# zhengfei0908/SBA-GAN

Hardware: AMD Instinct MI355X
Metric: images/sec (G+D step) at 256px (higher is better)
Workload: dtype bf16; 1 GPU; bird_style.yml 3-stage G+D step (64..256px), B=20 per GPU, G_NET variant=model, image_encoder=inception, text_encoder=RNN_ENCODER in the step; global_batch=20, parallelism=dp1, launch=replayer, losses_finite=True

## Files before the change

sba-gan_amd/csrc/encoder.hip:

```cpp
#include "common.h"

namespace {

__global__ void resize_fwd_kernel(const float* __restrict__ in, float* __restrict__ out, int NC, int S, int D) {
    const int64_t total = (int64_t)NC * D * D;
    const float sc = (float)(S - 1) / (float)(D - 1);
    for (int64_t i = blockIdx.x * (int64_t)blockDim.x + threadIdx.x; i < total; i += (int64_t)gridDim.x * blockDim.x) {
        const int x = (int)(i % D), y = (int)((i / D) % D);
        const int64_t nc = i / ((int64_t)D * D);
        const float fy = y * sc, fx = x * sc;
        int y0 = (int)fy, x0 = (int)fx;
        y0 = min(y0, S - 1); x0 = min(x0, S - 1);
        const int y1 = min(y0 + 1, S - 1), x1 = min(x0 + 1, S - 1);
        const float wy = fy - y0, wx = fx - x0;
        const float* p = in + nc * S * S;
        const float v = (1.f - wy) * ((1.f - wx) * p[y0 * S + x0] + wx * p[y0 * S + x1]) +
                        wy * ((1.f - wx) * p[y1 * S + x0] + wx * p[y1 * S + x1]);
        out[i] = v;
    }
}

__device__ __forceinline__ float resize_adj_w(int o, int r, float sc, int S) {
    const float f = o * sc;
    int i0 = (int)f;
    i0 = min(i0, S - 1);
    const int i1 = min(i0 + 1, S - 1);
    const float wgt = f - i0;
    return (i0 == r ? 1.f - wgt : 0.f) + (i1 == r ? wgt : 0.f);
}

__global__ void resize_bwd_kernel(const float* __restrict__ dout, float* __restrict__ din, int NC, int S, int D) {
    const int64_t total = (int64_t)NC * S * S;
    const float sc = (float)(S - 1) / (float)(D - 1);
    const float inv = 1.f / sc;
    for (int64_t i = blockIdx.x * (int64_t)blockDim.x + threadIdx.x; i < total; i += (int64_t)gridDim.x * blockDim.x) {
        const int c = (int)(i % S), r = (int)((i / S) % S);
        const int64_t nc = i / ((int64_t)S * S);
        const int ylo = max(0, (int)floorf((r - 1) * inv) - 1), yhi = min(D - 1, (int)ceilf((r + 1) * inv) + 1);
        const int xlo = max(0, (int)floorf((c - 1) * inv) - 1), xhi = min(D - 1, (int)ceilf((c + 1) * inv) + 1);
        const float* g = dout + nc * D * D;
        float acc = 0.f;
        for (int y = ylo; y <= yhi; ++y) {
            const float wy = resize_adj_w(y, r, sc, S);
            if (wy == 0.f) continue;
            float row = 0.f;
            for (int x = xlo; x <= xhi; ++x) {
                const float wx = resize_adj_w(x, c, sc, S);
                if (wx != 0.f) row += g[y * D + x] * wx;
            }
            acc += wy * row;
        }
        din[i] = acc;
    }
}

constexpr int RESIZE_MAXC = 4;
__global__ __launch_bounds__(256) void resize_bwd_tab_kernel(const float* __restrict__ dout, float* __restrict__ din, int NC,
                                                             int S, int D) {
    extern __shared__ unsigned char rs_lds[];
    int* t_o = reinterpret_cast<int*>(rs_lds);
    float* t_w = reinterpret_cast<float*>(rs_lds + (size_t)S * RESIZE_MAXC * 4);
    const float sc = (float)(S - 1) / (float)(D - 1);
    const float inv = 1.f / sc;
    for (int r = threadIdx.x; r < S; r += blockDim.x) {
        const int lo = max(0, (int)floorf((r - 1) * inv) - 1), hi = min(D - 1, (int)ceilf((r + 1) * inv) + 1);
        int k = 0;
        for (int o = lo; o <= hi && k < RESIZE_MAXC; ++o) {
            const float wgt = resize_adj_w(o, r, sc, S);
            if (wgt != 0.f) { t_o[r * RESIZE_MAXC + k] = o; t_w[r * RESIZE_MAXC + k] = wgt; ++k; }
        }
        for (; k < RESIZE_MAXC; ++k) { t_o[r * RESIZE_MAXC + k] = 0; t_w[r * RESIZE_MAXC + k] = 0.f; }
    }
    __syncthreads();
    const int64_t total = (int64_t)NC * S * S;
    for (int64_t i = blockIdx.x * (int64_t)blockDim.x + threadIdx.x; i < total; i += (int64_t)gridDim.x * blockDim.x) {
        const int c = (int)(i % S), r = (int)((i / S) % S);
        const int64_t nc = i / ((int64_t)S * S);
        const float* g = dout + nc * D * D;
        float acc = 0.f;
#pragma unroll
        for (int ky = 0; ky < RESIZE_MAXC; ++ky) {
            const float wy = t_w[r * RESIZE_MAXC + ky];
            if (wy == 0.f) continue;
            const float* grow = g + t_o[r * RESIZE_MAXC + ky] * D;
            float row = 0.f;
#pragma unroll
            for (int kx = 0; kx < RESIZE_MAXC; ++kx) {
                const float wx = t_w[c * RESIZE_MAXC + kx];
                if (wx != 0.f) row += grow[t_o[c * RESIZE_MAXC + kx]] * wx;
            }
            acc += wy * row;
        }
        din[i] = acc;
    }
}

template <typename T>
__global__ __launch_bounds__(256) void enc_stem_fwd_kernel(const float* __restrict__ img, const float* __restrict__ w,
                                                           const float* __restrict__ bias, T* __restrict__ out,
                                                           int N, int S, int O, int C) {
    constexpr int V = Vec16<T>::N;
    extern __shared__ float s_w[];
    for (int i = threadIdx.x; i < 27 * C; i += blockDim.x) {
        const int co = i / 27, k = i - co * 27;
        s_w[k * C + co] = w[i];
    }
    __syncthreads();
    const int cv = C / V;
    const int64_t total = (int64_t)N * O * O * cv;
    for (int64_t i = blockIdx.x * (int64_t)blockDim.x + threadIdx.x; i < total; i += (int64_t)gridDim.x * blockDim.x) {
        const int c = (int)(i % cv) * V;
        const int64_t p = i / cv;
        const int ox = (int)(p % O), oy = (int)((p / O) % O), n = (int)(p / ((int64_t)O * O));
        float acc[V];
#pragma unroll
        for (int k = 0; k < V; ++k) acc[k] = bias ? bias[c + k] : 0.f;
#pragma unroll
        for (int kh = 0; kh < 3; ++kh)
#pragma unroll
            for (int kw = 0; kw < 3; ++kw)
#pragma unroll
                for (int ci = 0; ci < 3; ++ci) {
                    const float v = img[(((int64_t)n * 3 + ci) * S + 2 * oy + kh) * S + 2 * ox + kw];
                    const float* wr = &s_w[((kh * 3 + kw) * 3 + ci) * C + c];
#pragma unroll
                    for (int k = 0; k < V; ++k) acc[k] += v * wr[k];
                }
        Vec16<T> o;
#pragma unroll
        for (int k = 0; k < V; ++k) o.set(k, bias ? fmaxf(acc[k], 0.f) : acc[k]);
        st16(out + p * C + c, o);
    }
}

template <typename T>
__global__ __launch_bounds__(256) void enc_stem_resize_fwd_kernel(const float* __restrict__ img, const float* __restrict__ w,
                                                                  const float* __restrict__ bias, T* __restrict__ out,
                                                                  int N, int S, int D, int O, int C) {
    constexpr int V = Vec16<T>::N;
    extern __shared__ float s_w[];
    for (int i = threadIdx.x; i < 27 * C; i += blockDim.x) {
        const int co = i / 27, k = i - co * 27;
        s_w[k * C + co] = w[i];
    }
    __syncthreads();
    const float sc = (float)(S - 1) / (float)(D - 1);
    const int cv = C / V;
    const int64_t total = (int64_t)N * O * O * cv;
    for (int64_t i = blockIdx.x * (int64_t)blockDim.x + threadIdx.x; i < total; i += (int64_t)gridDim.x * blockDim.x) {
        const int c = (int)(i % cv) * V;
        const int64_t p = i / cv;
        const int ox = (int)(p % O), oy = (int)((p / O) % O), n = (int)(p / ((int64_t)O * O));
        int x0[3], x1[3];
        float wx[3];
#pragma unroll
        for (int k = 0; k < 3; ++k) {
            const float fx = (2 * ox + k) * sc;
            x0[k] = min((int)fx, S - 1);
            x1[k] = min(x0[k] + 1, S - 1);
            wx[k] = fx - x0[k];
        }
        float acc[V];
#pragma unroll
        for (int k = 0; k < V; ++k) acc[k] = bias ? bias[c + k] : 0.f;
        const float* q0 = img + (int64_t)n * 3 * S * S;
#pragma unroll 1
        for (int kh = 0; kh < 3; ++kh) {
            const float fy = (2 * oy + kh) * sc;
            const int y0 = min((int)fy, S - 1), y1 = min(y0 + 1, S - 1);
            const float wy = fy - y0;
#pragma unroll
            for (int kw = 0; kw < 3; ++kw)
#pragma unroll
                for (int ci = 0; ci < 3; ++ci) {
                    const float* q = q0 + (int64_t)ci * S * S;
                    const float v = (1.f - wy) * ((1.f - wx[kw]) * q[y0 * S + x0[kw]] + wx[kw] * q[y0 * S + x1[kw]]) +
                                    wy * ((1.f - wx[kw]) * q[y1 * S + x0[kw]] + wx[kw] * q[y1 * S + x1[kw]]);
                    const float* wr = &s_w[((kh * 3 + kw) * 3 + ci) * C + c];
#pragma unroll
                    for (int k = 0; k < V; ++k) acc[k] += v * wr[k];
                }
        }
        Vec16<T> o;
#pragma unroll
        for (int k = 0; k < V; ++k) o.set(k, bias ? fmaxf(acc[k], 0.f) : acc[k]);
        st16(out + p * C + c, o);
    }
}

template <typename T>
__global__ __launch_bounds__(256) void enc_stem_bwd_kernel(const float* __restrict__ w, const T* __restrict__ out,
                                                           const T* __restrict__ dout, float* __restrict__ dimg,
                                                           int N, int S, int O, int C) {
    constexpr int V = Vec16<T>::N;
    extern __shared__ float s_w[];
    for (int i = threadIdx.x; i < 27 * C; i += blockDim.x) {
        const int co = i / 27, k = i - co * 27;
        s_w[k * C + co] = w[i];
    }
    __syncthreads();
    const int64_t total = (int64_t)N * S * S;
    for (int64_t p = blockIdx.x * (int64_t)blockDim.x + threadIdx.x; p < total; p += (int64_t)gridDim.x * blockDim.x) {
        const int ix = (int)(p % S), iy = (int)((p / S) % S), n = (int)(p / ((int64_t)S * S));
        float acc[3] = {0.f, 0.f, 0.f};
        for (int kh = iy & 1; kh < 3; kh += 2) {
            const int oy = (iy - kh) >> 1;
            if (iy - kh < 0 || oy >= O) continue;
            for (int kw = ix & 1; kw < 3; kw += 2) {
                const int ox = (ix - kw) >> 1;
                if (ix - kw < 0 || ox >= O) continue;
                const int64_t q = (((int64_t)n * O + oy) * O + ox) * C;
                for (int cv = 0; cv < C / V; ++cv) {
                    Vec16<T> ov = ld16(out + q + cv * V), dv = ld16(dout + q + cv * V);
#pragma unroll
                    for (int k = 0; k < V; ++k) {
                        const float dp = ov.get(k) > 0.f ? dv.get(k) : 0.f;
                        const int co = cv * V + k;
#pragma unroll
                        for (int ci = 0; ci < 3; ++ci) acc[ci] += dp * s_w[((kh * 3 + kw) * 3 + ci) * C + co];
                    }
                }
            }
        }
#pragma unroll
        for (int ci = 0; ci < 3; ++ci) dimg[(((int64_t)n * 3 + ci) * S + iy) * S + ix] = acc[ci];
    }
}

__global__ __launch_bounds__(256) void enc_stem_bwd_mfma_kernel(const float* __restrict__ w, const bf16_t* __restrict__ out,
                                                                const bf16_t* __restrict__ dout, float* __restrict__ dimg,
                                                                const int N, const int S, const int O, const int ntiles) {
    constexpr int C = 32;
    const int tid = threadIdx.x, lane = tid & 63, wid = tid >> 6;
    const int m = lane & 15, g = lane >> 4;
    bf16x8_t a_hi[4], a_lo[4];
    {
        const int ci = m >> 2, a = (m >> 1) & 1, b = m & 1;
#pragma unroll
        for (int t = 0; t < 4; ++t) {
            const int kh = a + 2 * (t >> 1), kw = b + 2 * (t & 1);
            const bool ok = m < 12 && kh < 3 && kw < 3;
            bf16x8_t hi, lo;
#pragma unroll
            for (int j = 0; j < 8; ++j) {
                const int co = 8 * g + j;
                const float v = ok ? w[co * 27 + (kh * 3 + kw) * 3 + ci] : 0.f;
                const bf16_t h = f2bf(v);
                hi[j] = (short)h;
                lo[j] = (short)f2bf(v - bf2f(h));
            }
            a_hi[t] = hi;
            a_lo[t] = lo;
        }
    }
    const int BH = (S + 1) / 2, tiles_x = (BH + 15) / 16;
    for (int tile = blockIdx.x * 4 + wid; tile < ntiles; tile += gridDim.x * 4) {
        const int txi = tile % tiles_x, by = (tile / tiles_x) % BH, n = tile / (tiles_x * BH);
        const int bx = txi * 16 + m;
        f32x4_t acc = f32x4_t{0.f, 0.f, 0.f, 0.f};
#pragma unroll
        for (int t = 0; t < 4; ++t) {
            const int oy = by - (t >> 1), ox = bx - (t & 1);
            uint4 dv = make_uint4(0, 0, 0, 0), ov = make_uint4(0, 0, 0, 0);
            if (oy >= 0 && oy < O && ox >= 0 && ox < O) {
                const int64_t q = (((int64_t)n * O + oy) * O + ox) * C + 8 * g;
                dv = *reinterpret_cast<const uint4*>(dout + q);
                ov = *reinterpret_cast<const uint4*>(out + q);
            }
            const uint32_t d[4] = {dv.x, dv.y, dv.z, dv.w}, o[4] = {ov.x, ov.y, ov.z, ov.w};
            bf16x8_t bfr;
#pragma unroll
            for (int k = 0; k < 4; ++k) {
                const uint32_t lo_ok = ((o[k] & 0x7fffu) != 0u && (o[k] & 0x8000u) == 0u) ? 0x0000ffffu : 0u;
                const uint32_t hi_ok = ((o[k] & 0x7fff0000u) != 0u && (o[k] & 0x80000000u) == 0u) ? 0xffff0000u : 0u;
                const uint32_t v = d[k] & (lo_ok | hi_ok);
                bfr[2 * k] = (short)(v & 0xffffu);
                bfr[2 * k + 1] = (short)(v >> 16);
            }
            acc = __builtin_amdgcn_mfma_f32_16x16x32_bf16(a_lo[t], bfr, acc, 0, 0, 0);
            acc = __builtin_amdgcn_mfma_f32_16x16x32_bf16(a_hi[t], bfr, acc, 0, 0, 0);
        }
        if (g < 3 && bx < BH) {
            float* o0 = dimg + (((int64_t)n * 3 + g) * S + 2 * by) * S + 2 * bx;
            const bool x1 = 2 * bx + 1 < S, y1 = 2 * by + 1 < S;
            o0[0] = acc[0];
            if (x1) o0[1] = acc[1];
            if (y1) {
                o0[S] = acc[2];
                if (x1) o0[S + 1] = acc[3];
            }
        }
    }
}

template <typename T>
__global__ void maxpool_fwd_kernel(const T* __restrict__ x, T* __restrict__ y, int N, int H, int W, int C, int xcs,
                                   int xco, int ycs, int yco) {
    constexpr int V = Vec16<T>::N;
    const int OH = (H - 3) / 2 + 1, OW = (W - 3) / 2 + 1, cv = C / V;
    const int64_t total = (int64_t)N * OH * OW * cv;
    for (int64_t i = blockIdx.x * (int64_t)blockDim.x + threadIdx.x; i < total; i += (int64_t)gridDim.x * blockDim.x) {
        const int c = (int)(i % cv) * V;
        const int64_t p = i / cv;
        const int ox = (int)(p % OW), oy = (int)((p / OW) % OH), n = (int)(p / ((int64_t)OW * OH));
        float m[V];
#pragma unroll
        for (int k = 0; k < V; ++k) m[k] = -INFINITY;
#pragma unroll
        for (int kh = 0; kh < 3; ++kh)
#pragma unroll
            for (int kw = 0; kw < 3; ++kw) {
                Vec16<T> v = ld16(x + (((int64_t)n * H + 2 * oy + kh) * W + 2 * ox + kw) * xcs + xco + c);
#pragma unroll
                for (int k = 0; k < V; ++k) m[k] = fmaxf(m[k], v.get(k));
            }
        Vec16<T> o;
#pragma unroll
        for (int k = 0; k < V; ++k) o.set(k, m[k]);
        st16(y + p * ycs + yco + c, o);
    }
}

template <typename T>
__global__ void maxpool_fwd_arg_kernel(const T* __restrict__ x, T* __restrict__ y, uint8_t* __restrict__ arg, int N,
                                       int H, int W, int C, int xcs, int xco, int ycs, int yco) {
    constexpr int V = Vec16<T>::N;
    const int OH = (H - 3) / 2 + 1, OW = (W - 3) / 2 + 1, cv = C / V;
    const int64_t total = (int64_t)N * OH * OW * cv;
    for (int64_t i = blockIdx.x * (int64_t)blockDim.x + threadIdx.x; i < total; i += (int64_t)gridDim.x * blockDim.x) {
        const int c = (int)(i % cv) * V;
        const int64_t p = i / cv;
        const int ox = (int)(p % OW), oy = (int)((p / OW) % OH), n = (int)(p / ((int64_t)OW * OH));
        float m[V];
        uint8_t a[V];
#pragma unroll
        for (int k = 0; k < V; ++k) { m[k] = -INFINITY; a[k] = 255; }
#pragma unroll
        for (int kh = 0; kh < 3; ++kh)
#pragma unroll
            for (int kw = 0; kw < 3; ++kw) {
                Vec16<T> v = ld16(x + (((int64_t)n * H + 2 * oy + kh) * W + 2 * ox + kw) * xcs + xco + c);
#pragma unroll
                for (int k = 0; k < V; ++k) {
                    const float f = v.get(k);
                    if (f > m[k]) { m[k] = f; a[k] = (uint8_t)(kh * 3 + kw); }
                }
            }
        Vec16<T> o;
#pragma unroll
        for (int k = 0; k < V; ++k) o.set(k, m[k]);
        st16(y + p * ycs + yco + c, o);
        uint8_t* ap = arg + p * C + c;
        if (V == 8) {
            uint2 w;
            w.x = a[0] | (a[1] << 8) | (a[2] << 16) | ((uint32_t)a[3] << 24);
            w.y = a[4] | (a[5] << 8) | (a[6] << 16) | ((uint32_t)a[7] << 24);
            *reinterpret_cast<uint2*>(ap) = w;
        } else {
            *reinterpret_cast<uint32_t*>(ap) = a[0] | (a[1] << 8) | (a[2] << 16) | ((uint32_t)a[3] << 24);
        }
    }
}

template <typename T>
__global__ void maxpool_bwd_arg_kernel(const uint8_t* __restrict__ arg, const T* __restrict__ dy, T* __restrict__ dx,
                                       int N, int H, int W, int C, int dycs, int dyco, int dxcs, int dxco,
                                       int accumulate, const T* __restrict__ relu_mask) {
    constexpr int V = Vec16<T>::N;
    const int OH = (H - 3) / 2 + 1, OW = (W - 3) / 2 + 1, cv = C / V;
    const int64_t total = (int64_t)N * H * W * cv;
    for (int64_t i = blockIdx.x * (int64_t)blockDim.x + threadIdx.x; i < total; i += (int64_t)gridDim.x * blockDim.x) {
        const int c = (int)(i % cv) * V;
        const int64_t p = i / cv;
        const int ix = (int)(p % W), iy = (int)((p / W) % H), n = (int)(p / ((int64_t)W * H));
        float g[V];
#pragma unroll
        for (int k = 0; k < V; ++k) g[k] = 0.f;
        for (int oy = max(0, (iy - 1) >> 1); oy <= min(OH - 1, iy >> 1); ++oy) {
            if (iy - 2 * oy > 2) continue;
            for (int ox = max(0, (ix - 1) >> 1); ox <= min(OW - 1, ix >> 1); ++ox) {
                if (ix - 2 * ox > 2) continue;
                const uint32_t mypos = (uint32_t)((iy - 2 * oy) * 3 + (ix - 2 * ox));
                const int64_t q = ((int64_t)n * OH + oy) * OW + ox;
                uint32_t aw[2] = {0u, 0u};
                if (V == 8) {
                    const uint2 w = *reinterpret_cast<const uint2*>(arg + q * C + c);
                    aw[0] = w.x; aw[1] = w.y;
                } else {
                    aw[0] = *reinterpret_cast<const uint32_t*>(arg + q * C + c);
                }
                Vec16<T> d = ld16(dy + q * dycs + dyco + c);
#pragma unroll
                for (int k = 0; k < V; ++k)
                    if (((aw[k >> 2] >> (8 * (k & 3))) & 255u) == mypos) g[k] += d.get(k);
            }
        }
        T* op = dx + p * dxcs + dxco + c;
        Vec16<T> o;
        if (accumulate) o = ld16(op);
#pragma unroll
        for (int k = 0; k < V; ++k) o.set(k, g[k] + (accumulate ? o.get(k) : 0.f));
        if (relu_mask) {
            const Vec16<T> m = ld16(relu_mask + p * dxcs + dxco + c);
#pragma unroll
            for (int k = 0; k < V; ++k) if (!(m.get(k) > 0.f)) o.set(k, 0.f);
        }
        st16(op, o);
    }
}

template <typename T>
__global__ void maxpool_bwd_kernel(const T* __restrict__ x, const T* __restrict__ dy, T* __restrict__ dx, int N, int H,
                                   int W, int C, int xcs, int xco, int dycs, int dyco, int dxcs, int dxco,
                                   int accumulate) {
    constexpr int V = Vec16<T>::N;
    const int OH = (H - 3) / 2 + 1, OW = (W - 3) / 2 + 1, cv = C / V;
    const int64_t total = (int64_t)N * H * W * cv;
    for (int64_t i = blockIdx.x * (int64_t)blockDim.x + threadIdx.x; i < total; i += (int64_t)gridDim.x * blockDim.x) {
        const int c = (int)(i % cv) * V;
        const int64_t p = i / cv;
        const int ix = (int)(p % W), iy = (int)((p / W) % H), n = (int)(p / ((int64_t)W * H));
        float g[V];
#pragma unroll
        for (int k = 0; k < V; ++k) g[k] = 0.f;
        for (int oy = max(0, (iy - 1) >> 1); oy <= min(OH - 1, iy >> 1); ++oy) {
            if (iy - 2 * oy > 2) continue;
            for (int ox = max(0, (ix - 1) >> 1); ox <= min(OW - 1, ix >> 1); ++ox) {
                if (ix - 2 * ox > 2) continue;
                const int mypos = (iy - 2 * oy) * 3 + (ix - 2 * ox);
                float m[V];
                int arg[V];
#pragma unroll
                for (int k = 0; k < V; ++k) { m[k] = -INFINITY; arg[k] = -1; }
#pragma unroll
                for (int kh = 0; kh < 3; ++kh)
#pragma unroll
                    for (int kw = 0; kw < 3; ++kw) {
                        Vec16<T> v = ld16(x + (((int64_t)n * H + 2 * oy + kh) * W + 2 * ox + kw) * xcs + xco + c);
#pragma unroll
                        for (int k = 0; k < V; ++k) {
                            const float f = v.get(k);
                            if (f > m[k]) { m[k] = f; arg[k] = kh * 3 + kw; }
                        }
                    }
                Vec16<T> d = ld16(dy + (((int64_t)n * OH + oy) * OW + ox) * dycs + dyco + c);
#pragma unroll
                for (int k = 0; k < V; ++k)
                    if (arg[k] == mypos) g[k] += d.get(k);
            }
        }
        T* op = dx + p * dxcs + dxco + c;
        Vec16<T> o;
        if (accumulate) o = ld16(op);
#pragma unroll
        for (int k = 0; k < V; ++k) o.set(k, g[k] + (accumulate ? o.get(k) : 0.f));
        st16(op, o);
    }
}

template <typename T>
__global__ void avgpool3_kernel(const T* __restrict__ x, T* __restrict__ y, int N, int H, int W, int C, int xcs,
                                int xco, int ycs, int yco, int accumulate) {
    constexpr int V = Vec16<T>::N;
    const int cv = C / V;
    const int64_t total = (int64_t)N * H * W * cv;
    for (int64_t i = blockIdx.x * (int64_t)blockDim.x + threadIdx.x; i < total; i += (int64_t)gridDim.x * blockDim.x) {
        const int c = (int)(i % cv) * V;
        const int64_t p = i / cv;
        const int ix = (int)(p % W), iy = (int)((p / W) % H), n = (int)(p / ((int64_t)W * H));
        float s[V];
#pragma unroll
        for (int k = 0; k < V; ++k) s[k] = 0.f;
#pragma unroll
        for (int dy = -1; dy <= 1; ++dy)
#pragma unroll
            for (int dx = -1; dx <= 1; ++dx) {
                const int yy = iy + dy, xx = ix + dx;
                if (yy < 0 || yy >= H || xx < 0 || xx >= W) continue;
                Vec16<T> v = ld16(x + (((int64_t)n * H + yy) * W + xx) * xcs + xco + c);
#pragma unroll
                for (int k = 0; k < V; ++k) s[k] += v.get(k);
            }
        T* op = y + p * ycs + yco + c;
        Vec16<T> o;
        if (accumulate) o = ld16(op);
#pragma unroll
        for (int k = 0; k < V; ++k) o.set(k, s[k] * (1.f / 9.f) + (accumulate ? o.get(k) : 0.f));
        st16(op, o);
    }
}

template <typename T>
__global__ void relu_bwd_kernel(const T* __restrict__ out, const T* __restrict__ dout, T* __restrict__ dpre,
                                int64_t rows, int C, int ocs, int oco, int dcs, int dco) {
    constexpr int V = Vec16<T>::N;
    const int cv = C / V;
    const int64_t total = rows * cv;
    for (int64_t i = blockIdx.x * (int64_t)blockDim.x + threadIdx.x; i < total; i += (int64_t)gridDim.x * blockDim.x) {
        const int c = (int)(i % cv) * V;
        const int64_t r = i / cv;
        Vec16<T> o = ld16(out + r * ocs + oco + c), d = ld16(dout + r * dcs + dco + c), q;
#pragma unroll
        for (int k = 0; k < V; ++k) q.set(k, o.get(k) > 0.f ? d.get(k) : 0.f);
        st16(dpre + r * C + c, q);
    }
}

template <typename T>
__global__ void gap_fwd_kernel(const T* __restrict__ x, float* __restrict__ y, int N, int HW, int C) {
    const int i = blockIdx.x * blockDim.x + threadIdx.x;
    if (i >= N * C) return;
    const int n = i / C, c = i - n * C;
    float s = 0.f;
    for (int p = 0; p < HW; ++p) s += to_f<T>(x[((int64_t)n * HW + p) * C + c]);
    y[i] = s / HW;
}
template <typename T>
__global__ __launch_bounds__(256) void gap_bwd_kernel(const float* __restrict__ dy, T* __restrict__ dx, int N, int HW, int C) {
    constexpr int V = Vec16<T>::N;
    const int cv = C / V;
    const int total = N * HW * cv;
    for (int i = blockIdx.x * blockDim.x + threadIdx.x; i < total; i += gridDim.x * blockDim.x) {
        const int r = i / cv, c = (i - r * cv) * V;
        const int n = r / HW;
        const float* src = dy + (int64_t)n * C + c;
        Vec16<T> q;
#pragma unroll
        for (int k = 0; k < V; ++k) q.set(k, src[k] / HW);
        st16(dx + (int64_t)r * C + c, q);
    }
}

template <typename T>
__global__ void nhwc_to_nchw_kernel(const T* __restrict__ x, float* __restrict__ y, int N, int HW, int C) {
    const int64_t total = (int64_t)N * HW * C;
    for (int64_t i = blockIdx.x * (int64_t)blockDim.x + threadIdx.x; i < total; i += (int64_t)gridDim.x * blockDim.x) {
        const int p = (int)(i % HW), c = (int)((i / HW) % C), n = (int)(i / ((int64_t)HW * C));
        y[i] = to_f<T>(x[((int64_t)n * HW + p) * C + c]);
    }
}
template <typename T>
__global__ void nchw_to_nhwc_kernel(const float* __restrict__ x, T* __restrict__ y, int N, int HW, int C) {
    const int64_t total = (int64_t)N * HW * C;
    for (int64_t i = blockIdx.x * (int64_t)blockDim.x + threadIdx.x; i < total; i += (int64_t)gridDim.x * blockDim.x) {
        const int c = (int)(i % C), p = (int)((i / C) % HW), n = (int)(i / ((int64_t)HW * C));
        y[i] = from_f<T>(x[((int64_t)n * C + c) * HW + p]);
    }
}

inline int grid_for(int64_t items, int cap = 8192) {
    int64_t b = (items + 255) / 256;
    if (b < 1) b = 1;
    return (int)(b > cap ? cap : b);
}
inline bool slice_ok(int dtype, int C, int cs, int co) {
    const int V = dtype == SBA_BF16 ? 8 : 4;
    return C > 0 && C % V == 0 && cs >= C + co && co >= 0 && cs % V == 0 && co % V == 0;
}

}

extern "C" int sba_resize_bilinear(const float* in, float* out, int NC, int S, int D, int backward, void* stream) {
    if (!in || !out || NC <= 0 || S < 2 || D < 2) return SBA_E_ARG;
    hipStream_t st = (hipStream_t)stream;
    if (!backward) {
        SBA_LAUNCH(resize_fwd_kernel, dim3(grid_for((int64_t)NC * D * D)), dim3(256), 0, st, in, out, NC, S, D);
    } else {
        if (D >= S && S >= 2 && S <= 2048 && 2 * (int64_t)(D - 1) <= 3 * (int64_t)(S - 1))
            SBA_LAUNCH(resize_bwd_tab_kernel, dim3(grid_for((int64_t)NC * S * S, 2048)), dim3(256), (size_t)S * RESIZE_MAXC * 8,
                       st, in, out, NC, S, D);
        else
        SBA_LAUNCH(resize_bwd_kernel, dim3(grid_for((int64_t)NC * S * S)), dim3(256), 0, st, in, out, NC, S, D);
    }
    return SBA_CHECK_LAUNCH();
}

extern "C" int sba_enc_stem_fwd(int dtype, const float* img, const float* w, const float* bias, void* out, int N,
                                int S, int C, void* stream) {
    if (!img || !w || !out || N <= 0 || S < 3 || C <= 0 || C % 8 || C > 256) return SBA_E_ARG;
    const int O = (S - 3) / 2 + 1, V = dtype == SBA_BF16 ? 8 : 4;
    SBA_DISPATCH(dtype, SBA_LAUNCH((enc_stem_fwd_kernel<T>), dim3(grid_for((int64_t)N * O * O * (C / V), 4096)),
                                           dim3(256), sizeof(float) * 27 * C, (hipStream_t)stream, img, w, bias,
                                           (T*)out, N, S, O, C));
    return SBA_CHECK_LAUNCH();
}

extern "C" int sba_enc_stem_bwd(int dtype, const float* w, const void* out, const void* dout, float* dimg, int N,
                                int S, int C, void* stream) {
    if (!w || !out || !dout || !dimg || N <= 0 || S < 3 || C <= 0 || C % 8 || C > 256) return SBA_E_ARG;
    const int O = (S - 3) / 2 + 1;
    if (dtype == SBA_BF16 && C == 32 && (((uintptr_t)out | (uintptr_t)dout) & 15) == 0) {
        const int BH = (S + 1) / 2, ntiles = N * BH * ((BH + 15) / 16);
        SBA_LAUNCH(enc_stem_bwd_mfma_kernel, dim3((ntiles + 3) / 4 < 8192 ? (ntiles + 3) / 4 : 8192), dim3(256), 0,
                   (hipStream_t)stream, w, (const bf16_t*)out, (const bf16_t*)dout, dimg, N, S, O, ntiles);
        return SBA_CHECK_LAUNCH();
    }
    SBA_DISPATCH(dtype, SBA_LAUNCH((enc_stem_bwd_kernel<T>), dim3(grid_for((int64_t)N * S * S, 4096)), dim3(256),
                                           sizeof(float) * 27 * C, (hipStream_t)stream, w, (const T*)out,
                                           (const T*)dout, dimg, N, S, O, C));
    return SBA_CHECK_LAUNCH();
}

extern "C" int sba_maxpool3x3s2_fwd(int dtype, const void* x, void* y, int N, int H, int W, int C, int xcs, int xco,
                                    int ycs, int yco, void* stream) {
    if (!x || !y || N <= 0 || H < 3 || W < 3 || !slice_ok(dtype, C, xcs, xco) || !slice_ok(dtype, C, ycs, yco))
        return SBA_E_ARG;
    const int OH = (H - 3) / 2 + 1, OW = (W - 3) / 2 + 1, V = dtype == SBA_BF16 ? 8 : 4;
    SBA_DISPATCH(dtype, SBA_LAUNCH((maxpool_fwd_kernel<T>), dim3(grid_for((int64_t)N * OH * OW * (C / V))),
                                           dim3(256), 0, (hipStream_t)stream, (const T*)x, (T*)y, N, H, W, C, xcs, xco,
                                           ycs, yco));
    return SBA_CHECK_LAUNCH();
}

extern "C" int sba_maxpool3x3s2_bwd(int dtype, const void* x, const void* dy, void* dx, int N, int H, int W, int C,
                                    int xcs, int xco, int dycs, int dyco, int dxcs, int dxco, int accumulate,
                                    void* stream) {
    if (!x || !dy || !dx || N <= 0 || H < 3 || W < 3 || !slice_ok(dtype, C, xcs, xco) ||
        !slice_ok(dtype, C, dycs, dyco) || !slice_ok(dtype, C, dxcs, dxco))
        return SBA_E_ARG;
    const int V = dtype == SBA_BF16 ? 8 : 4;
    SBA_DISPATCH(dtype, SBA_LAUNCH((maxpool_bwd_kernel<T>), dim3(grid_for((int64_t)N * H * W * (C / V))),
                                           dim3(256), 0, (hipStream_t)stream, (const T*)x, (const T*)dy, (T*)dx, N, H,
                                           W, C, xcs, xco, dycs, dyco, dxcs, dxco, accumulate));
    return SBA_CHECK_LAUNCH();
}

extern "C" int sba_maxpool3x3s2_fwd_arg(int dtype, const void* x, void* y, uint8_t* argmax, int N, int H, int W, int C,
                                        int xcs, int xco, int ycs, int yco, void* stream) {
    if (!x || !y || !argmax || N <= 0 || H < 3 || W < 3 || !slice_ok(dtype, C, xcs, xco) || !slice_ok(dtype, C, ycs, yco))
        return SBA_E_ARG;
    const int OH = (H - 3) / 2 + 1, OW = (W - 3) / 2 + 1, V = dtype == SBA_BF16 ? 8 : 4;
    if (((uintptr_t)argmax & 7) != 0) return SBA_E_ARG;
    SBA_DISPATCH(dtype, SBA_LAUNCH((maxpool_fwd_arg_kernel<T>), dim3(grid_for((int64_t)N * OH * OW * (C / V))),
                                           dim3(256), 0, (hipStream_t)stream, (const T*)x, (T*)y, argmax, N, H, W, C,
                                           xcs, xco, ycs, yco));
    return SBA_CHECK_LAUNCH();
}

extern "C" int sba_maxpool3x3s2_bwd_arg(int dtype, const uint8_t* argmax, const void* dy, void* dx, int N, int H, int W,
                                        int C, int dycs, int dyco, int dxcs, int dxco, int accumulate,
                                        const void* relu_mask, void* stream) {
    if (!argmax || !dy || !dx || N <= 0 || H < 3 || W < 3 || !slice_ok(dtype, C, dycs, dyco) ||
        !slice_ok(dtype, C, dxcs, dxco) || ((uintptr_t)argmax & 7) != 0)
        return SBA_E_ARG;
    const int V = dtype == SBA_BF16 ? 8 : 4;
    SBA_DISPATCH(dtype, SBA_LAUNCH((maxpool_bwd_arg_kernel<T>), dim3(grid_for((int64_t)N * H * W * (C / V))),
                                           dim3(256), 0, (hipStream_t)stream, argmax, (const T*)dy, (T*)dx, N, H, W, C,
                                           dycs, dyco, dxcs, dxco, accumulate, (const T*)relu_mask));
    return SBA_CHECK_LAUNCH();
}

extern "C" int sba_enc_stem_resize_fwd(int dtype, const float* img, const float* w, const float* bias, void* out, int N,
                                       int S, int D, int C, void* stream) {
    if (!img || !w || !out || N <= 0 || S < 2 || D < 3 || C <= 0 || C % 8 || C > 256) return SBA_E_ARG;
    const int O = (D - 3) / 2 + 1, V = dtype == SBA_BF16 ? 8 : 4;
    SBA_DISPATCH(dtype, SBA_LAUNCH((enc_stem_resize_fwd_kernel<T>), dim3(grid_for((int64_t)N * O * O * (C / V), 8192)),
                                           dim3(256), sizeof(float) * 27 * C, (hipStream_t)stream, img, w, bias, (T*)out, N,
                                           S, D, O, C));
    return SBA_CHECK_LAUNCH();
}

extern "C" int sba_avgpool3x3(int dtype, const void* x, void* y, int N, int H, int W, int C, int xcs, int xco,
                              int ycs, int yco, int accumulate, void* stream) {
    if (!x || !y || N <= 0 || H <= 0 || W <= 0 || !slice_ok(dtype, C, xcs, xco) || !slice_ok(dtype, C, ycs, yco))
        return SBA_E_ARG;
    const int V = dtype == SBA_BF16 ? 8 : 4;
    SBA_DISPATCH(dtype, SBA_LAUNCH((avgpool3_kernel<T>), dim3(grid_for((int64_t)N * H * W * (C / V))), dim3(256),
                                           0, (hipStream_t)stream, (const T*)x, (T*)y, N, H, W, C, xcs, xco, ycs, yco,
                                           accumulate));
    return SBA_CHECK_LAUNCH();
}

extern "C" int sba_relu_bwd(int dtype, const void* out, const void* dout, void* dpre, int64_t rows, int C, int ocs,
                            int oco, int dcs, int dco, void* stream) {
    if (!out || !dout || !dpre || rows <= 0 || !slice_ok(dtype, C, ocs, oco) || !slice_ok(dtype, C, dcs, dco))
        return SBA_E_ARG;
    const int V = dtype == SBA_BF16 ? 8 : 4;
    SBA_DISPATCH(dtype, SBA_LAUNCH((relu_bwd_kernel<T>), dim3(grid_for(rows * (C / V))), dim3(256), 0,
                                           (hipStream_t)stream, (const T*)out, (const T*)dout, (T*)dpre, rows, C, ocs,
                                           oco, dcs, dco));
    return SBA_CHECK_LAUNCH();
}

extern "C" int sba_global_avgpool(int dtype, void* x, float* y, int N, int HW, int C, int backward, void* stream) {
    if (!x || !y || N <= 0 || HW <= 0 || C <= 0) return SBA_E_ARG;
    if (!backward) {
        SBA_DISPATCH(dtype, SBA_LAUNCH((gap_fwd_kernel<T>), dim3(cdiv((int64_t)N * C, 256)), dim3(256), 0,
                                               (hipStream_t)stream, (const T*)x, y, N, HW, C));
    } else {
        if (C % 8 != 0 || (int64_t)N * HW * C >= (1ll << 31)) return SBA_E_ARG;
        SBA_DISPATCH(dtype, SBA_LAUNCH((gap_bwd_kernel<T>), dim3(grid_for((int64_t)N * HW * C / (dtype == SBA_BF16 ? 8 : 4))), dim3(256), 0,
                                               (hipStream_t)stream, (const float*)y, (T*)x, N, HW, C));
    }
    return SBA_CHECK_LAUNCH();
}

extern "C" int sba_layout_nhwc_nchw(int dtype, void* nhwc, float* nchw, int N, int HW, int C, int to_nhwc, void* stream) {
    if (!nhwc || !nchw || N <= 0 || HW <= 0 || C <= 0) return SBA_E_ARG;
    if (!to_nhwc) {
        SBA_DISPATCH(dtype, SBA_LAUNCH((nhwc_to_nchw_kernel<T>), dim3(grid_for((int64_t)N * HW * C)), dim3(256), 0,
                                               (hipStream_t)stream, (const T*)nhwc, nchw, N, HW, C));
    } else {
        SBA_DISPATCH(dtype, SBA_LAUNCH((nchw_to_nhwc_kernel<T>), dim3(grid_for((int64_t)N * HW * C)), dim3(256), 0,
                                               (hipStream_t)stream, (const float*)nchw, (T*)nhwc, N, HW, C));
    }
    return SBA_CHECK_LAUNCH();
}
```

Baseline: 2097 images/sec.

## Rework encoder pooling, global-avgpool and layout kernels for cheaper indexing and coalescing

Four encoder kernels are rewritten. Maxpool backward now uses a 3D grid over (n, row, width×channel) with incremental index walking instead of 64-bit div/mod, and it loads its four candidate windows directly. Avgpool3 now computes runs of 4 outputs from a shared 3×6 register window so neighbouring loads are reused. Global average pooling becomes vectorized and unrolled, and the NHWC/NCHW layout conversion becomes a shared-memory tiled transpose. The aim is to cut index arithmetic and uncoalesced traffic in the inception encoder, at the cost of more registers and extra grid-shape logic.

```diff
diff --git a/sba-gan_amd/csrc/encoder.hip b/sba-gan_amd/csrc/encoder.hip
--- a/sba-gan_amd/csrc/encoder.hip
+++ b/sba-gan_amd/csrc/encoder.hip
@@ -293,6 +293,26 @@
     }
 }
 
+constexpr int POOL_GRID_X = 256, POOL_GRID_YZ = 65535;
+struct PoolWalk {
+    uint32_t q, c, dq, dc;
+    __device__ __forceinline__ explicit PoolWalk(uint32_t cv) {
+        const uint32_t i = blockIdx.x * blockDim.x + threadIdx.x, st = gridDim.x * blockDim.x;
+        q = i / cv; c = i - q * cv;
+        dq = st / cv; dc = st - dq * cv;
+    }
+    __device__ __forceinline__ void next(uint32_t cv) {
+        q += dq; c += dc;
+        if (c >= cv) { c -= cv; ++q; }
+    }
+};
+template <typename T> __device__ __forceinline__ Vec16<T> zero16() {
+    Vec16<T> r;
+#pragma unroll
+    for (int k = 0; k < Vec16<T>::N; ++k) r.set(k, 0.f);
+    return r;
+}
+
 template <typename T>
 __global__ void maxpool_fwd_kernel(const T* __restrict__ x, T* __restrict__ y, int N, int H, int W, int C, int xcs,
                                    int xco, int ycs, int yco) {
@@ -363,50 +383,66 @@
 }
 
 template <typename T>
-__global__ void maxpool_bwd_arg_kernel(const uint8_t* __restrict__ arg, const T* __restrict__ dy, T* __restrict__ dx,
-                                       int N, int H, int W, int C, int dycs, int dyco, int dxcs, int dxco,
-                                       int accumulate, const T* __restrict__ relu_mask) {
+__global__ __launch_bounds__(256) void maxpool_bwd_arg_kernel(const uint8_t* __restrict__ arg, const T* __restrict__ dy,
+                                                              T* __restrict__ dx, int N, int H, int W, int C, int dycs, int dyco,
+                                                              int dxcs, int dxco, int accumulate, const T* __restrict__ relu_mask) {
     constexpr int V = Vec16<T>::N;
-    const int OH = (H - 3) / 2 + 1, OW = (W - 3) / 2 + 1, cv = C / V;
-    const int64_t total = (int64_t)N * H * W * cv;
-    for (int64_t i = blockIdx.x * (int64_t)blockDim.x + threadIdx.x; i < total; i += (int64_t)gridDim.x * blockDim.x) {
-        const int c = (int)(i % cv) * V;
-        const int64_t p = i / cv;
-        const int ix = (int)(p % W), iy = (int)((p / W) % H), n = (int)(p / ((int64_t)W * H));
-        float g[V];
-#pragma unroll
-        for (int k = 0; k < V; ++k) g[k] = 0.f;
-        for (int oy = max(0, (iy - 1) >> 1); oy <= min(OH - 1, iy >> 1); ++oy) {
-            if (iy - 2 * oy > 2) continue;
-            for (int ox = max(0, (ix - 1) >> 1); ox <= min(OW - 1, ix >> 1); ++ox) {
-                if (ix - 2 * ox > 2) continue;
-                const uint32_t mypos = (uint32_t)((iy - 2 * oy) * 3 + (ix - 2 * ox));
-                const int64_t q = ((int64_t)n * OH + oy) * OW + ox;
-                uint32_t aw[2] = {0u, 0u};
-                if (V == 8) {
-                    const uint2 w = *reinterpret_cast<const uint2*>(arg + q * C + c);
-                    aw[0] = w.x; aw[1] = w.y;
-                } else {
-                    aw[0] = *reinterpret_cast<const uint32_t*>(arg + q * C + c);
+    const int OH = (H - 3) / 2 + 1, OW = (W - 3) / 2 + 1;
+    const uint32_t cv = C / V;
+    for (int n = blockIdx.z; n < N; n += gridDim.z)
+        for (int iy = blockIdx.y; iy < H; iy += gridDim.y) {
+            const int oys[2] = {(iy - 1) >> 1, iy >> 1};
+            const bool yok[2] = {oys[0] >= 0 && oys[0] < OH, (iy & 1) == 0 && oys[1] < OH};
+            for (PoolWalk it(cv); it.q < (uint32_t)W; it.next(cv)) {
+                const int ix = (int)it.q, c = (int)it.c * V;
+                const int oxs[2] = {(ix - 1) >> 1, ix >> 1};
+                const bool xok[2] = {oxs[0] >= 0 && oxs[0] < OW, (ix & 1) == 0 && oxs[1] < OW};
+                uint32_t aw[2][2][2];
+                Vec16<T> d[2][2];
+#pragma unroll
+                for (int a = 0; a < 2; ++a)
+#pragma unroll
+                    for (int b = 0; b < 2; ++b) {
+                        aw[a][b][0] = aw[a][b][1] = 0xffffffffu;
+                        d[a][b] = zero16<T>();
+                        if (yok[a] && xok[b]) {
+                            const int64_t q = ((int64_t)n * OH + oys[a]) * OW + oxs[b];
+                            if (V == 8) {
+                                const uint2 w = *reinterpret_cast<const uint2*>(arg + q * C + c);
+                                aw[a][b][0] = w.x; aw[a][b][1] = w.y;
+                            } else {
+                                aw[a][b][0] = *reinterpret_cast<const uint32_t*>(arg + q * C + c);
+                            }
+                            d[a][b] = ld16(dy + q * dycs + dyco + c);
+                        }
+                    }
+                const int64_t p = ((int64_t)n * H + iy) * W + ix;
+                T* op = dx + p * dxcs + dxco + c;
+                Vec16<T> o = zero16<T>(), m = zero16<T>();
+                if (accumulate) o = ld16(op);
+                if (relu_mask) m = ld16(relu_mask + p * dxcs + dxco + c);
+                float g[V];
+#pragma unroll
+                for (int k = 0; k < V; ++k) g[k] = 0.f;
+#pragma unroll
+                for (int a = 0; a < 2; ++a)
+#pragma unroll
+                    for (int b = 0; b < 2; ++b) {
+                        if (!(yok[a] && xok[b])) continue;
+                        const uint32_t mypos = (uint32_t)((iy - 2 * oys[a]) * 3 + (ix - 2 * oxs[b]));
+#pragma unroll
+                        for (int k = 0; k < V; ++k)
+                            if (((aw[a][b][k >> 2] >> (8 * (k & 3))) & 255u) == mypos) g[k] += d[a][b].get(k);
+                    }
+#pragma unroll
+                for (int k = 0; k < V; ++k) o.set(k, g[k] + (accumulate ? o.get(k) : 0.f));
+                if (relu_mask) {
+#pragma unroll
+                    for (int k = 0; k < V; ++k) if (!(m.get(k) > 0.f)) o.set(k, 0.f);
                 }
-                Vec16<T> d = ld16(dy + q * dycs + dyco + c);
-#pragma unroll
-                for (int k = 0; k < V; ++k)
-                    if (((aw[k >> 2] >> (8 * (k & 3))) & 255u) == mypos) g[k] += d.get(k);
-            }
-        }
-        T* op = dx + p * dxcs + dxco + c;
-        Vec16<T> o;
-        if (accumulate) o = ld16(op);
-#pragma unroll
-        for (int k = 0; k < V; ++k) o.set(k, g[k] + (accumulate ? o.get(k) : 0.f));
-        if (relu_mask) {
-            const Vec16<T> m = ld16(relu_mask + p * dxcs + dxco + c);
-#pragma unroll
-            for (int k = 0; k < V; ++k) if (!(m.get(k) > 0.f)) o.set(k, 0.f);
-        }
-        st16(op, o);
-    }
+                st16(op, o);
+            }
+        }
 }
 
 template <typename T>
@@ -458,36 +494,55 @@
     }
 }
 
-template <typename T>
-__global__ void avgpool3_kernel(const T* __restrict__ x, T* __restrict__ y, int N, int H, int W, int C, int xcs,
-                                int xco, int ycs, int yco, int accumulate) {
-    constexpr int V = Vec16<T>::N;
-    const int cv = C / V;
-    const int64_t total = (int64_t)N * H * W * cv;
-    for (int64_t i = blockIdx.x * (int64_t)blockDim.x + threadIdx.x; i < total; i += (int64_t)gridDim.x * blockDim.x) {
-        const int c = (int)(i % cv) * V;
-        const int64_t p = i / cv;
-        const int ix = (int)(p % W), iy = (int)((p / W) % H), n = (int)(p / ((int64_t)W * H));
-        float s[V];
-#pragma unroll
-        for (int k = 0; k < V; ++k) s[k] = 0.f;
-#pragma unroll
-        for (int dy = -1; dy <= 1; ++dy)
-#pragma unroll
-            for (int dx = -1; dx <= 1; ++dx) {
-                const int yy = iy + dy, xx = ix + dx;
-                if (yy < 0 || yy >= H || xx < 0 || xx >= W) continue;
-                Vec16<T> v = ld16(x + (((int64_t)n * H + yy) * W + xx) * xcs + xco + c);
-#pragma unroll
-                for (int k = 0; k < V; ++k) s[k] += v.get(k);
-            }
-        T* op = y + p * ycs + yco + c;
-        Vec16<T> o;
-        if (accumulate) o = ld16(op);
-#pragma unroll
-        for (int k = 0; k < V; ++k) o.set(k, s[k] * (1.f / 9.f) + (accumulate ? o.get(k) : 0.f));
-        st16(op, o);
-    }
+constexpr int AVG_RUN = 4;
+template <typename T>
+__global__ __launch_bounds__(256) void avgpool3_kernel(const T* __restrict__ x, T* __restrict__ y, int N, int H, int W, int C,
+                                                       int xcs, int xco, int ycs, int yco, int accumulate) {
+    constexpr int V = Vec16<T>::N, R = AVG_RUN;
+    const uint32_t cv = C / V, runs = ((uint32_t)W + R - 1) / R;
+    for (int n = blockIdx.z; n < N; n += gridDim.z)
+        for (int iy = blockIdx.y; iy < H; iy += gridDim.y) {
+            const int64_t row = ((int64_t)n * H + iy) * W;
+            for (PoolWalk it(cv); it.q < runs; it.next(cv)) {
+                const int x0 = (int)it.q * R, c = (int)it.c * V;
+                Vec16<T> v[3][R + 2], old[R];
+#pragma unroll
+                for (int r = 0; r < 3; ++r)
+#pragma unroll
+                    for (int j = 0; j < R + 2; ++j) {
+                        const int yy = iy + r - 1, xx = x0 + j - 1;
+                        v[r][j] = yy >= 0 && yy < H && xx >= 0 && xx < W
+                                      ? ld16(x + (row + (int64_t)(r - 1) * W + xx) * xcs + xco + c) : zero16<T>();
+                    }
+                T* op = y + (row + x0) * ycs + yco + c;
+#pragma unroll
+                for (int j = 0; j < R; ++j) old[j] = accumulate && x0 + j < W ? ld16(op + (int64_t)j * ycs) : zero16<T>();
+                float f[3][R + 2][V];
+#pragma unroll
+                for (int r = 0; r < 3; ++r)
+#pragma unroll
+                    for (int j = 0; j < R + 2; ++j)
+#pragma unroll
+                        for (int k = 0; k < V; ++k) f[r][j][k] = v[r][j].get(k);
+#pragma unroll
+                for (int j = 0; j < R; ++j) {
+                    if (x0 + j >= W) break;
+                    float s[V];
+#pragma unroll
+                    for (int k = 0; k < V; ++k) s[k] = 0.f;
+#pragma unroll
+                    for (int r = 0; r < 3; ++r)
+#pragma unroll
+                        for (int d = 0; d < 3; ++d)
+#pragma unroll
+                            for (int k = 0; k < V; ++k) s[k] += f[r][j + d][k];
+                    Vec16<T> o;
+#pragma unroll
+                    for (int k = 0; k < V; ++k) o.set(k, s[k] * (1.f / 9.f) + (accumulate ? old[j].get(k) : 0.f));
+                    st16(op + (int64_t)j * ycs, o);
+                }
+            }
+        }
 }
 
 template <typename T>
@@ -506,14 +561,49 @@
     }
 }
 
-template <typename T>
-__global__ void gap_fwd_kernel(const T* __restrict__ x, float* __restrict__ y, int N, int HW, int C) {
-    const int i = blockIdx.x * blockDim.x + threadIdx.x;
-    if (i >= N * C) return;
-    const int n = i / C, c = i - n * C;
-    float s = 0.f;
-    for (int p = 0; p < HW; ++p) s += to_f<T>(x[((int64_t)n * HW + p) * C + c]);
-    y[i] = s / HW;
+constexpr int GAP_AHEAD = 32;
+template <typename T, int VEC> struct GapLoad {
+    Vec16<T> v;
+    __device__ __forceinline__ void load(const T* p) { v = ld16(p); }
+    __device__ __forceinline__ float get(int k) const { return v.get(k); }
+};
+template <typename T> struct GapLoad<T, 1> {
+    T v;
+    __device__ __forceinline__ void load(const T* p) { v = *p; }
+    __device__ __forceinline__ float get(int) const { return to_f<T>(v); }
+};
+template <typename T, int VEC>
+__global__ __launch_bounds__(64) void gap_fwd_kernel(const T* __restrict__ x, float* __restrict__ y, int N, int HW, int C) {
+    constexpr int U = GAP_AHEAD;
+    const int cvn = C / VEC;
+    for (int n = blockIdx.y; n < N; n += gridDim.y)
+        for (int ci = blockIdx.x * blockDim.x + threadIdx.x; ci < cvn; ci += gridDim.x * blockDim.x) {
+            const T* xp = x + (int64_t)n * HW * C + (int64_t)ci * VEC;
+            float s[VEC];
+#pragma unroll
+            for (int k = 0; k < VEC; ++k) s[k] = 0.f;
+            for (int p0 = 0; p0 < HW; p0 += U) {
+                GapLoad<T, VEC> v[U];
+#pragma unroll
+                for (int j = 0; j < U; ++j)
+                    if (p0 + j < HW) v[j].load(xp + (int64_t)(p0 + j) * C);
+#pragma unroll
+                for (int j = 0; j < U; ++j)
+                    if (p0 + j < HW) {
+#pragma unroll
+                        for (int k = 0; k < VEC; ++k) s[k] += v[j].get(k);
+                    }
+            }
+            float* yp = y + (int64_t)n * C + (int64_t)ci * VEC;
+#pragma unroll
+            for (int k = 0; k < VEC; ++k) s[k] = s[k] / HW;
+            if (VEC == 1) {
+                yp[0] = s[0];
+            } else {
+#pragma unroll
+                for (int k = 0; k < VEC; k += 4) *reinterpret_cast<float4*>(yp + k) = make_float4(s[k], s[k + 1], s[k + 2], s[k + 3]);
+            }
+        }
 }
 template <typename T>
 __global__ __launch_bounds__(256) void gap_bwd_kernel(const float* __restrict__ dy, T* __restrict__ dx, int N, int HW, int C) {
@@ -531,27 +621,61 @@
     }
 }
 
-template <typename T>
-__global__ void nhwc_to_nchw_kernel(const T* __restrict__ x, float* __restrict__ y, int N, int HW, int C) {
-    const int64_t total = (int64_t)N * HW * C;
-    for (int64_t i = blockIdx.x * (int64_t)blockDim.x + threadIdx.x; i < total; i += (int64_t)gridDim.x * blockDim.x) {
-        const int p = (int)(i % HW), c = (int)((i / HW) % C), n = (int)(i / ((int64_t)HW * C));
-        y[i] = to_f<T>(x[((int64_t)n * HW + p) * C + c]);
-    }
-}
-template <typename T>
-__global__ void nchw_to_nhwc_kernel(const float* __restrict__ x, T* __restrict__ y, int N, int HW, int C) {
-    const int64_t total = (int64_t)N * HW * C;
-    for (int64_t i = blockIdx.x * (int64_t)blockDim.x + threadIdx.x; i < total; i += (int64_t)gridDim.x * blockDim.x) {
-        const int c = (int)(i % C), p = (int)((i / C) % HW), n = (int)(i / ((int64_t)HW * C));
-        y[i] = from_f<T>(x[((int64_t)n * C + c) * HW + p]);
-    }
+constexpr int LAY_P = 32, LAY_C = 64;
+template <typename T, bool TO_NHWC>
+__global__ __launch_bounds__(256) void layout_kernel(T* __restrict__ nhwc, float* __restrict__ nchw, int N, int HW, int C) {
+    __shared__ float tile[LAY_P][LAY_C + 1];
+    const int tid = threadIdx.x;
+    const int cl = tid & 63, pr = tid >> 6;
+    const int pl = tid & 31, cr = ((tid >> 5) & 1) * 32 + (tid >> 6);
+    const int c0 = blockIdx.x * LAY_C;
+    for (int n = blockIdx.z; n < N; n += gridDim.z)
+        for (int p0 = blockIdx.y * LAY_P; p0 < HW; p0 += gridDim.y * LAY_P) {
+            T* hp = nhwc + ((int64_t)n * HW + p0 + pr) * C + c0 + cl;
+            float* cp = nchw + ((int64_t)n * C + c0 + cr) * HW + p0 + pl;
+            const bool hc = c0 + cl < C, cpix = p0 + pl < HW;
+            if (!TO_NHWC) {
+                T v[8];
+#pragma unroll
+                for (int j = 0; j < 8; ++j)
+                    if (hc && p0 + pr + 4 * j < HW) v[j] = hp[(int64_t)4 * j * C];
+#pragma unroll
+                for (int j = 0; j < 8; ++j)
+                    if (hc && p0 + pr + 4 * j < HW) tile[pr + 4 * j][cl] = to_f<T>(v[j]);
+                __syncthreads();
+#pragma unroll
+                for (int j = 0; j < 8; ++j)
+                    if (cpix && c0 + cr + 4 * j < C) cp[(int64_t)4 * j * HW] = tile[pl][cr + 4 * j];
+            } else {
+                float v[8];
+#pragma unroll
+                for (int j = 0; j < 8; ++j)
+                    if (cpix && c0 + cr + 4 * j < C) v[j] = cp[(int64_t)4 * j * HW];
+#pragma unroll
+                for (int j = 0; j < 8; ++j)
+                    if (cpix && c0 + cr + 4 * j < C) tile[pl][cr + 4 * j] = v[j];
+                __syncthreads();
+#pragma unroll
+                for (int j = 0; j < 8; ++j)
+                    if (hc && p0 + pr + 4 * j < HW) hp[(int64_t)4 * j * C] = from_f<T>(tile[pr + 4 * j][cl]);
+            }
+            __syncthreads();
+        }
 }
 
 inline int grid_for(int64_t items, int cap = 8192) {
     int64_t b = (items + 255) / 256;
     if (b < 1) b = 1;
     return (int)(b > cap ? cap : b);
+}
+inline dim3 pool_grid(int64_t row_items, int rows, int N) {
+    const int64_t bx = (row_items + 255) / 256;
+    return dim3((unsigned)(bx > POOL_GRID_X ? POOL_GRID_X : bx), (unsigned)(rows > POOL_GRID_YZ ? POOL_GRID_YZ : rows),
+                (unsigned)(N > POOL_GRID_YZ ? POOL_GRID_YZ : N));
+}
+inline dim3 pool_block(int64_t row_items) {
+    const int64_t bx = (row_items + 255) / 256, per = (row_items + bx - 1) / bx;
+    return dim3(bx > POOL_GRID_X ? 256u : (unsigned)((per + 63) / 64 * 64));
 }
 inline bool slice_ok(int dtype, int C, int cs, int co) {
     const int V = dtype == SBA_BF16 ? 8 : 4;
@@ -644,8 +768,8 @@
         !slice_ok(dtype, C, dxcs, dxco) || ((uintptr_t)argmax & 7) != 0)
         return SBA_E_ARG;
     const int V = dtype == SBA_BF16 ? 8 : 4;
-    SBA_DISPATCH(dtype, SBA_LAUNCH((maxpool_bwd_arg_kernel<T>), dim3(grid_for((int64_t)N * H * W * (C / V))),
-                                           dim3(256), 0, (hipStream_t)stream, argmax, (const T*)dy, (T*)dx, N, H, W, C,
+    SBA_DISPATCH(dtype, SBA_LAUNCH((maxpool_bwd_arg_kernel<T>), pool_grid((int64_t)W * (C / V), H, N),
+                                           pool_block((int64_t)W * (C / V)), 0, (hipStream_t)stream, argmax, (const T*)dy, (T*)dx, N, H, W, C,
                                            dycs, dyco, dxcs, dxco, accumulate, (const T*)relu_mask));
     return SBA_CHECK_LAUNCH();
 }
@@ -665,8 +789,8 @@
     if (!x || !y || N <= 0 || H <= 0 || W <= 0 || !slice_ok(dtype, C, xcs, xco) || !slice_ok(dtype, C, ycs, yco))
         return SBA_E_ARG;
     const int V = dtype == SBA_BF16 ? 8 : 4;
-    SBA_DISPATCH(dtype, SBA_LAUNCH((avgpool3_kernel<T>), dim3(grid_for((int64_t)N * H * W * (C / V))), dim3(256),
-                                           0, (hipStream_t)stream, (const T*)x, (T*)y, N, H, W, C, xcs, xco, ycs, yco,
+    SBA_DISPATCH(dtype, SBA_LAUNCH((avgpool3_kernel<T>), pool_grid((int64_t)cdiv(W, AVG_RUN) * (C / V), H, N),
+                                           pool_block((int64_t)cdiv(W, AVG_RUN) * (C / V)), 0, (hipStream_t)stream, (const T*)x, (T*)y, N, H, W, C, xcs, xco, ycs, yco,
                                            accumulate));
     return SBA_CHECK_LAUNCH();
 }
@@ -685,8 +809,14 @@
 extern "C" int sba_global_avgpool(int dtype, void* x, float* y, int N, int HW, int C, int backward, void* stream) {
     if (!x || !y || N <= 0 || HW <= 0 || C <= 0) return SBA_E_ARG;
     if (!backward) {
-        SBA_DISPATCH(dtype, SBA_LAUNCH((gap_fwd_kernel<T>), dim3(cdiv((int64_t)N * C, 256)), dim3(256), 0,
-                                               (hipStream_t)stream, (const T*)x, y, N, HW, C));
+        const int V = dtype == SBA_BF16 ? 8 : 4;
+        const dim3 gy((unsigned)(N > POOL_GRID_YZ ? POOL_GRID_YZ : N));
+        if (C % V == 0 && (((uintptr_t)x | (uintptr_t)y) & 15) == 0)
+            SBA_DISPATCH(dtype, SBA_LAUNCH((gap_fwd_kernel<T, Vec16<T>::N>), dim3(cdiv(C / V, 64), gy.x), dim3(64), 0,
+                                                   (hipStream_t)stream, (const T*)x, y, N, HW, C));
+        else
+            SBA_DISPATCH(dtype, SBA_LAUNCH((gap_fwd_kernel<T, 1>), dim3(cdiv(C, 64), gy.x), dim3(64), 0,
+                                                   (hipStream_t)stream, (const T*)x, y, N, HW, C));
     } else {
         if (C % 8 != 0 || (int64_t)N * HW * C >= (1ll << 31)) return SBA_E_ARG;
         SBA_DISPATCH(dtype, SBA_LAUNCH((gap_bwd_kernel<T>), dim3(grid_for((int64_t)N * HW * C / (dtype == SBA_BF16 ? 8 : 4))), dim3(256), 0,
@@ -697,12 +827,14 @@
 
 extern "C" int sba_layout_nhwc_nchw(int dtype, void* nhwc, float* nchw, int N, int HW, int C, int to_nhwc, void* stream) {
     if (!nhwc || !nchw || N <= 0 || HW <= 0 || C <= 0) return SBA_E_ARG;
+    const int py = cdiv(HW, LAY_P);
+    const dim3 grid(cdiv(C, LAY_C), (unsigned)(py > POOL_GRID_YZ ? POOL_GRID_YZ : py), (unsigned)(N > POOL_GRID_YZ ? POOL_GRID_YZ : N));
     if (!to_nhwc) {
-        SBA_DISPATCH(dtype, SBA_LAUNCH((nhwc_to_nchw_kernel<T>), dim3(grid_for((int64_t)N * HW * C)), dim3(256), 0,
-                                               (hipStream_t)stream, (const T*)nhwc, nchw, N, HW, C));
+        SBA_DISPATCH(dtype, SBA_LAUNCH((layout_kernel<T, false>), grid, dim3(256), 0, (hipStream_t)stream, (T*)nhwc, nchw, N,
+                                               HW, C));
     } else {
-        SBA_DISPATCH(dtype, SBA_LAUNCH((nchw_to_nhwc_kernel<T>), dim3(grid_for((int64_t)N * HW * C)), dim3(256), 0,
-                                               (hipStream_t)stream, (const float*)nchw, (T*)nhwc, N, HW, C));
-    }
-    return SBA_CHECK_LAUNCH();
-}
+        SBA_DISPATCH(dtype, SBA_LAUNCH((layout_kernel<T, true>), grid, dim3(256), 0, (hipStream_t)stream, (T*)nhwc, nchw, N,
+                                               HW, C));
+    }
+    return SBA_CHECK_LAUNCH();
+}
```

Result: no change. 2110 images/sec, median of 6 (+0.6%).
